# cheneeheng/2s-AGCN

Hardware: AMD Instinct MI355X
Metric: skeleton-clips/sec fwd+bwd, NTU (N,3,300,25,2) (higher is better)
Workload: dtype f32; 1 GPU; AGCN joint-stream NTU-xview shape, full training step (fwd, CE, bwd, grad all-reduce, clip 1.0, SGD nesterov); per_gpu_batch=64, global_batch=64, input=(N,3,300,25,2), parallelism=dp1, bn=per-replica

## Files before the change

### 2s-agcn_amd/csrc/conv_gemm_bf16.hip

```cpp
#include "agcn_common.h"
#include "epilogue.h"
#include "gate.h"
#include "split_f16.h"

namespace {

typedef __bf16 bf16x8 __attribute__((ext_vector_type(8)));
typedef __bf16 bf16x2 __attribute__((ext_vector_type(2)));
typedef float f32x2 __attribute__((ext_vector_type(2)));
typedef unsigned u32x4 __attribute__((ext_vector_type(4)));
typedef f32x4 f32x4_u __attribute__((aligned(4)));

constexpr int CK = 16, NW = 8, NT = 512;

struct BfArgs {
  const float* in;
  const unsigned short* wp;
  const float* bias;
  float* out;
  float* stats;
  const float* add1;
  const float* mask1;
  const float* add2;
  const float* mask2;
  int N, M, Kinner, in_rows;
  int V, T_src, T_out, tt, ntiles;
  int src_stride, f_off;
  int out_fs, out_fo, T_full;
  int FW, WLR;
  int accumulate;
  int nchunks, nmb;
  int off_b;
  int off_bias;
  int dbg;
  int relu;
  const float* in_absmax;
};

struct GateBfArgs : BfArgs {
  GateArgs gate;
  int off_gate;
};
template <bool GATE> struct BfArgsOf { typedef BfArgs type; };
template <> struct BfArgsOf<true> { typedef GateBfArgs type; };

struct BfPackArgs {
  const float* w;
  unsigned short* wp;
  int M, Kinner, nchunks;
  long sa_m, sa_c;
  int tap_mul, tap_add, tap_flip_from;
};

__device__ __forceinline__ unsigned pack_bf16(float a, float b) {
  f32x2 v = {a, b};
  bf16x2 p = __builtin_convertvector(v, bf16x2);
  return __builtin_bit_cast(unsigned, p);
}
__device__ __forceinline__ float lo_as_f32(unsigned p) { return __builtin_bit_cast(float, p << 16); }
__device__ __forceinline__ float hi_as_f32(unsigned p) { return __builtin_bit_cast(float, p & 0xffff0000u); }

__device__ __forceinline__ void split_pair(float a, float b, unsigned& ph, unsigned& pm, unsigned& pl) {
  ph = pack_bf16(a, b);
  const float ra = a - lo_as_f32(ph), rb = b - hi_as_f32(ph);
  pm = pack_bf16(ra, rb);
  pl = pack_bf16(ra - lo_as_f32(pm), rb - hi_as_f32(pm));
}

template <bool F16>
__device__ __forceinline__ f32x16 mfma_split(bf16x8 x, bf16x8 y, f32x16 c) {
  if constexpr (F16)
    return __builtin_amdgcn_mfma_f32_32x32x16_f16(__builtin_bit_cast(f16x8, x), __builtin_bit_cast(f16x8, y), c, 0, 0, 0);
  else
    return __builtin_amdgcn_mfma_f32_32x32x16_bf16(x, y, c, 0, 0, 0);
}

template <int TAPS, int BM, bool F16 = false>
__global__ void __launch_bounds__(256) pack_weights_bf16_kernel(const BfPackArgs p) {
  constexpr int PER_PLANE = TAPS * 2 * BM * 8;
  const int ch = blockIdx.x % p.nchunks, mb = blockIdx.x / p.nchunks;
  unsigned short* dst = p.wp + (long)blockIdx.x * 3 * PER_PLANE;
  for (int e = threadIdx.x; e < PER_PLANE / 2; e += 256) {
    const int j = (e & 3) * 2;
    const int ml = (e >> 2) % BM;
    const int r = (e >> 2) / BM;
    const int h = r & 1, tap = r >> 1;
    const int m = mb * BM + ml;
    const int gt = p.tap_flip_from >= 0 ? (p.tap_flip_from - (tap * p.tap_mul + p.tap_add)) : tap;
    float v[2];
#pragma unroll
    for (int q = 0; q < 2; ++q) {
      const int kc = ch * CK + h * 8 + j + q;
      v[q] = (m < p.M && kc < p.Kinner) ? p.w[(long)m * p.sa_m + (long)kc * p.sa_c + gt] : 0.f;
    }
    unsigned ph, pm, pl = 0;
    if constexpr (F16) split_pair_f16(v[0] * F16_W_SCALE, v[1] * F16_W_SCALE, ph, pm);
    else split_pair(v[0], v[1], ph, pm, pl);
    const int o = ((tap * 2 + h) * BM + ml) * 8 + j;
    *reinterpret_cast<unsigned*>(dst + 0 * PER_PLANE + o) = ph;
    *reinterpret_cast<unsigned*>(dst + 1 * PER_PLANE + o) = pm;
    *reinterpret_cast<unsigned*>(dst + 2 * PER_PLANE + o) = pl;
  }
}

template <int TAPS, int NPL, int WQ, int TM, int TN = 1, bool F16 = false, bool GATE = false>
__global__ void __launch_bounds__(NT, (TAPS == 1 && TM == 2 && TN == 1) ? 4 : 2) conv_gemm_bf16_kernel(const typename BfArgsOf<GATE>::type a) {
  constexpr int BM = TM * 32;
  constexpr int A_PLANE = TAPS * 2 * BM * 16;
  constexpr int A4 = NPL * A_PLANE / 16;
  constexpr int EA = (A4 + NT - 1) / NT;
  extern __shared__ __attribute__((aligned(16))) unsigned char smem[];
  unsigned char* Ab = smem;
  unsigned char* Bb = smem + a.off_b;

  const int tid = threadIdx.x, lane = tid & 63;
  const int wave = __builtin_amdgcn_readfirstlane(tid >> 6);
  const int lr = lane & 31, h = lane >> 5;
  const int bid = xcd_remap(blockIdx.x, gridDim.x);
  const int mbk = bid % a.nmb;
  const int nt_id = bid / a.nmb;
  const int n = nt_id / a.ntiles, tile_id = nt_id - n * a.ntiles;
  const int m0 = mbk * BM;
  const int V = a.V, tt = a.tt, t0 = tile_id * tt;
  const int ttv = tt * V;
  const int nvalid = min(tt, a.T_out - t0) * V;
  const int Psrc = a.T_src * V;
  const int f0 = t0 * a.src_stride + a.f_off;
  const int WL = a.FW * V, WLR = a.WLR;
  const int g0 = f0 * V;
  float rs_s = 1.f, rs_inv = 1.f;
  if constexpr (F16) { f16_range_scale(a.in_absmax, rs_s, rs_inv); rs_inv *= F16_W_INV; }

  int boff[TN];
#pragma unroll
  for (int tn = 0; tn < TN; ++tn) {
    int q = (wave * TN + tn) * 32 + lr;
    if (q >= ttv) q = 0;
    const int tl = q / V;
    boff[tn] = tl * a.src_stride * V + (q - tl * V);
  }

  float* bias_s = reinterpret_cast<float*>(smem + a.off_bias);
  for (int e = tid; e < BM; e += NT) bias_s[e] = (a.bias && m0 + e < a.M) ? a.bias[m0 + e] : 0.f;

  f32x16 acc[TM][TN];
#pragma unroll
  for (int tm = 0; tm < TM; ++tm)
#pragma unroll
    for (int tn = 0; tn < TN; ++tn)
#pragma unroll
      for (int j = 0; j < 16; ++j) acc[tm][tn][j] = 0.f;

  const int hb = wave & 1, wq = wave >> 1;
  const int qlen = (WL + 3) >> 2;
  u32x4 ra[EA];
  float rb[WQ][8];
  const int KP = a.nchunks * CK;
  const float* gl = nullptr;
  float gpos[WQ];
  if constexpr (GATE) {
    gl = reinterpret_cast<const float*>(smem + a.off_gate);
    gate_stage<NT>(reinterpret_cast<float*>(smem + a.off_gate), a.gate, n, V, a.T_src, a.Kinner, f0, a.FW, KP);
    __syncthreads();
#pragma unroll
    for (int u = 0; u < WQ; ++u) {
      const int rr = lane + 64 * u;
      gpos[u] = rr < qlen ? gate_pos(gl, KP, wq * qlen + rr, V, WL) : 0.f;
    }
    if constexpr (F16) {
      if (a.in_absmax) {
        f16_range_scale_of<14>(*a.in_absmax * gate_bound(gl, KP, a.FW, lane), rs_s, rs_inv);
        rs_inv *= F16_W_INV;
      }
    }
  }
  const u32x4* wp4 = reinterpret_cast<const u32x4*>(a.wp) + (long)mbk * a.nchunks * (3 * A_PLANE / 16);

  auto issue_loads = [&](int ch) __attribute__((always_inline)) {
    const u32x4* src = wp4 + (long)ch * (3 * A_PLANE / 16);
#pragma unroll
    for (int u = 0; u < EA; ++u) ra[u] = src[min(tid + u * NT, A4 - 1)];
    const int kc0 = ch * CK + hb * 8;
#pragma unroll
    for (int u = 0; u < WQ; ++u) {
      const int rr = lane + 64 * u;
      const int r = wq * qlen + rr;
      const int gp = g0 + r;
      const bool okp = rr < qlen && r < WL && gp >= 0 && gp < Psrc;
#pragma unroll
      for (int c = 0; c < 8; ++c) {
        const bool ok = okp && (kc0 + c) < a.Kinner;
        rb[u][c] = a.in[((long)n * a.in_rows + (ok ? (kc0 + c) : 0)) * Psrc + (ok ? gp : 0)];
      }
    }
  };
  auto commit_lds = [&](int ch) __attribute__((always_inline)) {
#pragma unroll
    for (int u = 0; u < EA; ++u)
      if (tid + u * NT < A4) reinterpret_cast<u32x4*>(Ab)[tid + u * NT] = ra[u];
    const int kc0 = ch * CK + hb * 8;
#pragma unroll
    for (int u = 0; u < WQ; ++u) {
      const int rr = lane + 64 * u;
      const int r = wq * qlen + rr;
      const int gp = g0 + r;
      const bool okp = rr < qlen && r < WL && gp >= 0 && gp < Psrc;
      u32x4 ph, pm, pl;
#pragma unroll
      for (int c = 0; c < 4; ++c) {
        float x0 = (okp && (kc0 + 2 * c) < a.Kinner) ? rb[u][2 * c] : 0.f;
        float x1 = (okp && (kc0 + 2 * c + 1) < a.Kinner) ? rb[u][2 * c + 1] : 0.f;
        if constexpr (GATE) {
          x0 = x0 * gpos[u] * gl[kc0 + 2 * c];
          x1 = x1 * gpos[u] * gl[kc0 + 2 * c + 1];
        }
        unsigned a0, a1, a2 = 0;
        if constexpr (F16) split_pair_f16(x0 * rs_s, x1 * rs_s, a0, a1);
        else split_pair(x0, x1, a0, a1, a2);
        ph[c] = a0; pm[c] = a1; pl[c] = a2;
      }
      if (rr < qlen && r < WL) {
        *reinterpret_cast<u32x4*>(Bb + ((0 * 2 + hb) * WLR + r) * 16) = ph;
        if (NPL >= 2) *reinterpret_cast<u32x4*>(Bb + ((1 * 2 + hb) * WLR + r) * 16) = pm;
        if (NPL == 3) *reinterpret_cast<u32x4*>(Bb + ((2 * 2 + hb) * WLR + r) * 16) = pl;
      }
    }
  };

  const int nchunks = a.nchunks;
  if (nchunks > 0) issue_loads(0);
  for (int ch = 0; ch < nchunks; ++ch) {
    __syncthreads();
    if (!(a.dbg & 2) || ch == 0) {
      commit_lds(ch);
      if (ch + 1 < nchunks) issue_loads(ch + 1);
    }
    __syncthreads();
    if (a.dbg & 1) continue;
    bf16x8 afc[NPL], bfc[NPL][TN];
    auto load_a = [&](bf16x8 (&af)[NPL], int tap, int tm) __attribute__((always_inline)) {
#pragma unroll
      for (int pl = 0; pl < NPL; ++pl)
        af[pl] = *reinterpret_cast<const bf16x8*>(Ab + pl * A_PLANE + (((tap * 2 + h) * BM) + tm * 32 + lr) * 16);
    };
    auto load_b = [&](bf16x8 (&bf)[NPL][TN], int tap) __attribute__((always_inline)) {
#pragma unroll
      for (int pl = 0; pl < NPL; ++pl)
#pragma unroll
        for (int tn = 0; tn < TN; ++tn)
          bf[pl][tn] = *reinterpret_cast<const bf16x8*>(Bb + ((pl * 2 + h) * WLR + boff[tn] + tap * V) * 16);
    };
    load_b(bfc, 0);
    load_a(afc, 0, 0);
    __builtin_amdgcn_sched_group_barrier(0x100, NPL * (TN + 1), 0);
#pragma unroll 1
    for (int tap = 0; tap < TAPS; ++tap) {
      bf16x8 bfn[NPL][TN];
      const int tapn = min(tap + 1, TAPS - 1);
#pragma unroll
      for (int tm = 0; tm < TM; ++tm) {
        bf16x8 afn[NPL];
        load_a(afn, tm + 1 == TM ? tapn : tap, tm + 1 == TM ? 0 : tm + 1);
        if (tm + 1 == TM) load_b(bfn, tapn);
#pragma unroll
        for (int tn = 0; tn < TN; ++tn) {
          if (NPL == 3) {
            acc[tm][tn] = mfma_split<F16>(afc[NPL - 1], bfc[0][tn], acc[tm][tn]);
            acc[tm][tn] = mfma_split<F16>(afc[0], bfc[NPL - 1][tn], acc[tm][tn]);
            acc[tm][tn] = mfma_split<F16>(afc[NPL >= 2 ? 1 : 0], bfc[NPL >= 2 ? 1 : 0][tn], acc[tm][tn]);
          }
          if (NPL >= 2) {
            acc[tm][tn] = mfma_split<F16>(afc[NPL >= 2 ? 1 : 0], bfc[0][tn], acc[tm][tn]);
            acc[tm][tn] = mfma_split<F16>(afc[0], bfc[NPL >= 2 ? 1 : 0][tn], acc[tm][tn]);
          }
          acc[tm][tn] = mfma_split<F16>(afc[0], bfc[0][tn], acc[tm][tn]);
        }
        __builtin_amdgcn_sched_group_barrier(0x100, NPL, 0);
        if (tm + 1 == TM) __builtin_amdgcn_sched_group_barrier(0x100, NPL * TN, 0);
        __builtin_amdgcn_sched_group_barrier(0x008, TN * (NPL == 3 ? 6 : NPL == 2 ? 3 : 1), 0);
#pragma unroll
        for (int pl = 0; pl < NPL; ++pl) afc[pl] = afn[pl];
      }
#pragma unroll
      for (int pl = 0; pl < NPL; ++pl)
#pragma unroll
        for (int tn = 0; tn < TN; ++tn) bfc[pl][tn] = bfn[pl][tn];
    }
  }

  if ((a.dbg & 4) && acc[0][0][0] != 12345.f) return;
  __syncthreads();
  float* tile = reinterpret_cast<float*>(smem);
  const int TP = NW * TN * 32 + 1;
  float* red = tile + BM * TP;
#pragma unroll
  for (int tm = 0; tm < TM; ++tm)
#pragma unroll
    for (int tn = 0; tn < TN; ++tn)
#pragma unroll
      for (int j = 0; j < 16; ++j)
        tile[(tm * 32 + mfma_row(j, h)) * TP + (wave * TN + tn) * 32 + lr] = F16 ? acc[tm][tn][j] * rs_inv : acc[tm][tn][j];
  __syncthreads();
  int poff[4 * TN];
#pragma unroll
  for (int u = 0; u < 4 * TN; ++u) {
    const int q2 = lane + 64 * u;
    const int tl2 = q2 / V;
    poff[u] = tl2 * a.out_fs * V + (q2 - tl2 * V);
  }
  EpiPtrs ep;
  ep.out = a.out; ep.add1 = a.add1; ep.mask1 = a.mask1; ep.add2 = a.add2; ep.mask2 = a.mask2; ep.stats = a.stats;
  ep.accumulate = a.accumulate; ep.relu = a.relu;
  const long Pfull = (long)a.T_full * V;
  const long rows0 = (long)n * a.M * Pfull + ((long)t0 * a.out_fs + a.out_fo) * V;
  epilogue_rows<BM, NW, 4 * TN>(ep, tile, TP, bias_s, red, a.M, m0, rows0, Pfull, nvalid, poff, (long)n * a.ntiles + tile_id);
}


template <int TAPS, int NPL, int R, int NWP = 4, bool F16 = false, bool GATE = false>
__global__ void __launch_bounds__((8 + NWP) * 64, 3) conv_pc_kernel(const typename BfArgsOf<GATE>::type a) {
  constexpr int TM = 4, BM = 128, NWC = 8, NTALL = (NWC + NWP) * 64, NTP = NWP * 64;
  constexpr int SLOT = NPL * 2 * BM * 16;
  constexpr int PIECES = SLOT / 1024;
  constexpr int PPW = (PIECES + NWP - 1) / NWP;
  constexpr int NMF = NPL == 3 ? 6 : NPL == 2 ? 3 : 1;
  extern __shared__ __attribute__((aligned(16))) unsigned char smem[];
  unsigned char* ring = smem;
  const int WLR = a.WLR, V = a.V;
  const int B_BYTES = NPL * 2 * WLR * 16;
  unsigned char* Bbase = smem + a.off_b;

  const int wave = __builtin_amdgcn_readfirstlane(threadIdx.x >> 6);
  const int lane = threadIdx.x & 63;
  const int bid = xcd_remap(blockIdx.x, gridDim.x);
  const int mbk = bid % a.nmb;
  const int nt_id = bid / a.nmb;
  const int n = nt_id / a.ntiles, tile_id = nt_id - n * a.ntiles;
  const int m0 = mbk * BM;
  const int tt = a.tt, t0 = tile_id * tt;
  const int ttv = tt * V;
  const int nvalid = min(tt, a.T_out - t0) * V;
  const int Psrc = a.T_src * V;
  const int g0 = (t0 + a.f_off) * V;
  const int WL = a.FW * V;
  const int nchunks = a.nchunks;
  const int G = nchunks * TAPS;
  float rs_s = 1.f, rs_inv = 1.f;
  if constexpr (F16) { f16_range_scale(a.in_absmax, rs_s, rs_inv); rs_inv *= F16_W_INV; }

  float* bias_s = reinterpret_cast<float*>(smem + a.off_bias);
  for (int e = threadIdx.x; e < BM; e += NTALL) bias_s[e] = (a.bias && m0 + e < a.M) ? a.bias[m0 + e] : 0.f;
  const int KP = nchunks * CK;
  const float* gl = nullptr;
  if constexpr (GATE) {
    gl = reinterpret_cast<const float*>(smem + a.off_gate);
    gate_stage<NTALL>(reinterpret_cast<float*>(smem + a.off_gate), a.gate, n, V, a.T_src, a.Kinner, t0 + a.f_off, a.FW, KP);
    __syncthreads();
    if constexpr (F16) {
      if (a.in_absmax) {
        f16_range_scale_of<14>(*a.in_absmax * gate_bound(gl, KP, a.FW, lane), rs_s, rs_inv);
        rs_inv *= F16_W_INV;
      }
    }
  }

  auto step_barrier = [&]() __attribute__((always_inline)) {
    asm volatile("s_waitcnt lgkmcnt(0)\n\ts_barrier" ::: "memory");
  };

  if (wave >= NWC) {
    const int pw = wave - NWC;
    typedef const __attribute__((address_space(1))) void* gptr_t;
    typedef __attribute__((address_space(3))) void* lptr_t;
    const unsigned char* wsrc = reinterpret_cast<const unsigned char*>(a.wp) + (long)mbk * G * SLOT + lane * 16;
    auto dma_slot = [&](int g) __attribute__((always_inline)) {
      const unsigned char* src = wsrc + (long)g * SLOT;
      unsigned char* dst = ring + (g % R) * SLOT;
#pragma unroll
      for (int u = 0; u < PPW; ++u) {
        const int piece = pw + u * NWP;
        if (piece < PIECES)
          __builtin_amdgcn_global_load_lds((gptr_t)(src + piece * 1024), (lptr_t)(dst + piece * 1024), 16, 0, 0);
      }
    };
    const int ptid = threadIdx.x - NWC * 64;
    const int npiece = (WL + 3) >> 2;
    const int ntask = 2 * npiece;
    constexpr int TK = 256 / NTP;
    f32x4 rb[TK][8];
    auto issue_B = [&](int ch) __attribute__((always_inline)) {
#pragma unroll
      for (int k = 0; k < TK; ++k) {
        if (k * NTP >= ntask) continue;
        int task = ptid + k * NTP;
        if (task >= ntask) task = ntask - 1;
        const int hb = task & 1, r0 = (task >> 1) * 4;
        const int gp = g0 + r0;
        const float* src = a.in + ((long)n * a.in_rows + ch * CK + hb * 8) * Psrc + gp;
        if (gp >= 0 && gp + 3 < Psrc) {
#pragma unroll
          for (int c = 0; c < 8; ++c) rb[k][c] = *reinterpret_cast<const f32x4_u*>(src + (long)c * Psrc);
        } else {
#pragma unroll
          for (int c = 0; c < 8; ++c)
#pragma unroll
            for (int e = 0; e < 4; ++e) {
              const bool ok = gp + e >= 0 && gp + e < Psrc;
              const float t = src[(long)c * Psrc + (ok ? e : -gp)];
              rb[k][c][e] = ok ? t : 0.f;
            }
        }
      }
    };
    float gpos[TK][4];
    if constexpr (GATE) {
#pragma unroll
      for (int k = 0; k < TK; ++k) {
        int task = ptid + k * NTP;
        if (task >= ntask) task = ntask - 1;
#pragma unroll
        for (int e = 0; e < 4; ++e) gpos[k][e] = (k * NTP < ntask) ? gate_pos(gl, KP, (task >> 1) * 4 + e, V, WL) : 0.f;
      }
    }
    auto commit_B = [&](unsigned char* Bb, int ch) __attribute__((always_inline)) {
#pragma unroll
      for (int k = 0; k < TK; ++k) {
        if (k * NTP >= ntask) continue;
        int task = ptid + k * NTP;
        if (task >= ntask) task = ntask - 1;
        const int hb = task & 1, r0 = (task >> 1) * 4;
        float gch[8];
        if constexpr (GATE) {
          const f32x4 g0v = *reinterpret_cast<const f32x4*>(gl + ch * CK + hb * 8);
          const f32x4 g1v = *reinterpret_cast<const f32x4*>(gl + ch * CK + hb * 8 + 4);
#pragma unroll
          for (int c = 0; c < 4; ++c) { gch[c] = g0v[c]; gch[4 + c] = g1v[c]; }
        }
#pragma unroll
        for (int e = 0; e < 4; ++e) {
          u32x4 ph, pm, pl;
#pragma unroll
          for (int c = 0; c < 4; ++c) {
            unsigned q0, q1, q2 = 0;
            float x0 = rb[k][2 * c][e], x1 = rb[k][2 * c + 1][e];
            if constexpr (GATE) {
              x0 = x0 * gpos[k][e] * gch[2 * c];
              x1 = x1 * gpos[k][e] * gch[2 * c + 1];
            }
            if constexpr (F16) split_pair_f16(x0 * rs_s, x1 * rs_s, q0, q1);
            else split_pair(x0, x1, q0, q1, q2);
            ph[c] = q0; pm[c] = q1; pl[c] = q2;
          }
          const int r = r0 + e;
          if (r < WLR) {
            *reinterpret_cast<u32x4*>(Bb + ((0 * 2 + hb) * WLR + r) * 16) = ph;
            if (NPL >= 2) *reinterpret_cast<u32x4*>(Bb + ((1 * 2 + hb) * WLR + r) * 16) = pm;
            if (NPL == 3) *reinterpret_cast<u32x4*>(Bb + ((2 * 2 + hb) * WLR + r) * 16) = pl;
          }
        }
      }
    };
#pragma unroll
    for (int g = 0; g < R - 1; ++g)
      if (g < G) dma_slot(g);
    issue_B(0);
    commit_B(Bbase, 0);
    asm volatile("s_waitcnt vmcnt(0)" ::: "memory");
    step_barrier();
    int g = 0;
    for (int ch = 0; ch < nchunks; ++ch) {
#pragma unroll
      for (int tap = 0; tap < TAPS; ++tap, ++g) {
        if (a.dbg & 2) { step_barrier(); continue; }
        if (g + R - 1 < G && !(a.dbg & 8)) dma_slot(g + R - 1);
        if (TAPS >= 3) {
          if (tap == 0 && ch + 1 < nchunks && !(a.dbg & 4)) issue_B(ch + 1);
          if (tap == (TAPS >= 6 ? TAPS - 3 : TAPS - 2) && ch + 1 < nchunks && !(a.dbg & 4))
            commit_B(Bbase + ((ch + 1) & 1) * B_BYTES, ch + 1);
        } else {
          if (tap == 0 && ch + 1 < nchunks) { issue_B(ch + 1); commit_B(Bbase + ((ch + 1) & 1) * B_BYTES, ch + 1); }
        }
        if (g + R - 1 < G) asm volatile("s_waitcnt vmcnt(%0)" :: "n"(PPW * (R - 3)) : "memory");
        else asm volatile("s_waitcnt vmcnt(0)" ::: "memory");
        step_barrier();
      }
    }
    return;
  }

  const int lr = lane & 31, h = lane >> 5;
  int q = wave * 32 + lr;
  if (q >= ttv) q = 0;
  const int boff = q;
  f32x16 acc[TM];
#pragma unroll
  for (int tm = 0; tm < TM; ++tm)
#pragma unroll
    for (int j = 0; j < 16; ++j) acc[tm][j] = 0.f;

  const unsigned char* a_lane = ring + (h * BM + lr) * 16;
  auto load_a = [&](bf16x8 (&af)[NPL], int slot, int tm) __attribute__((always_inline)) {
#pragma unroll
    for (int pl = 0; pl < NPL; ++pl)
      af[pl] = *reinterpret_cast<const bf16x8*>(a_lane + slot * SLOT + (pl * 2 * BM + tm * 32) * 16);
  };
  auto load_b = [&](bf16x8 (&bf)[NPL], const unsigned char* Bb, int tap) __attribute__((always_inline)) {
#pragma unroll
    for (int pl = 0; pl < NPL; ++pl)
      bf[pl] = *reinterpret_cast<const bf16x8*>(Bb + ((pl * 2 + h) * WLR + boff + tap * V) * 16);
  };
  step_barrier();
  bf16x8 afc[NPL], bfc[NPL];
  load_b(bfc, Bbase, 0);
  load_a(afc, 0, 0);
  int slot = 0;
  for (int ch = 0; ch < nchunks; ++ch) {
    const unsigned char* Bb = Bbase + (ch & 1) * B_BYTES;
    const unsigned char* Bn = Bbase + ((ch + 1) & 1) * B_BYTES;
#pragma unroll
    for (int tap = 0; tap < TAPS; ++tap) {
      const int slot_n = (slot + 1 == R) ? 0 : slot + 1;
      if (a.dbg & 1) { step_barrier(); continue; }
      bf16x8 bfn[NPL];
#pragma unroll
      for (int tm = 0; tm < TM; ++tm) {
        bf16x8 afn[NPL];
        if (tm + 1 < TM) {
          load_a(afn, slot, tm + 1);
        } else {
          load_a(afn, slot_n, 0);
          if (tap + 1 < TAPS) load_b(bfn, Bb, tap + 1);
          else load_b(bfn, Bn, 0);
        }
        if (NPL == 3) {
          acc[tm] = mfma_split<F16>(afc[NPL - 1], bfc[0], acc[tm]);
          acc[tm] = mfma_split<F16>(afc[0], bfc[NPL - 1], acc[tm]);
          acc[tm] = mfma_split<F16>(afc[NPL >= 2 ? 1 : 0], bfc[NPL >= 2 ? 1 : 0], acc[tm]);
        }
        if (NPL >= 2) {
          acc[tm] = mfma_split<F16>(afc[NPL >= 2 ? 1 : 0], bfc[0], acc[tm]);
          acc[tm] = mfma_split<F16>(afc[0], bfc[NPL >= 2 ? 1 : 0], acc[tm]);
        }
        acc[tm] = mfma_split<F16>(afc[0], bfc[0], acc[tm]);
        __builtin_amdgcn_sched_group_barrier(0x100, NPL, 0);
        if (tm + 1 == TM) __builtin_amdgcn_sched_group_barrier(0x100, NPL, 0);
        __builtin_amdgcn_sched_group_barrier(0x008, NMF, 0);
#pragma unroll
        for (int pl = 0; pl < NPL; ++pl) afc[pl] = afn[pl];
      }
#pragma unroll
      for (int pl = 0; pl < NPL; ++pl) bfc[pl] = bfn[pl];
      slot = slot_n;
      step_barrier();
    }
  }

  float* tile = reinterpret_cast<float*>(smem);
  const int TP = NWC * 32 + 1;
  float* red = tile + BM * TP;
#pragma unroll
  for (int tm = 0; tm < TM; ++tm)
#pragma unroll
    for (int j = 0; j < 16; ++j) tile[(tm * 32 + mfma_row(j, h)) * TP + wave * 32 + lr] = F16 ? acc[tm][j] * rs_inv : acc[tm][j];
  __syncthreads();
  int poff[4];
#pragma unroll
  for (int u = 0; u < 4; ++u) {
    const int q2 = lane + 64 * u;
    const int tl2 = q2 / V;
    poff[u] = tl2 * a.out_fs * V + (q2 - tl2 * V);
  }
  EpiPtrs ep;
  ep.out = a.out; ep.add1 = a.add1; ep.mask1 = a.mask1; ep.add2 = a.add2; ep.mask2 = a.mask2; ep.stats = a.stats;
  ep.accumulate = a.accumulate; ep.relu = a.relu;
  const long Pfull = (long)a.T_full * V;
  const long rows0 = (long)n * a.M * Pfull + ((long)t0 * a.out_fs + a.out_fo) * V;
  epilogue_rows<BM, NWC, 4>(ep, tile, TP, bias_s, red, a.M, m0, rows0, Pfull, nvalid, poff, (long)n * a.ntiles + tile_id);
}

template <int TAPS, int BM, int NPL, bool F16 = false>
__global__ void __launch_bounds__(256) pack_weights_slots_kernel(const BfPackArgs p) {
  constexpr int PLANE = 2 * BM * 8;
  const int tap = blockIdx.x % TAPS;
  const int ch = (blockIdx.x / TAPS) % p.nchunks, mb = blockIdx.x / (TAPS * p.nchunks);
  unsigned short* dst = p.wp + (long)blockIdx.x * NPL * PLANE;
  const int gt = p.tap_flip_from >= 0 ? (p.tap_flip_from - (tap * p.tap_mul + p.tap_add)) : tap;
  for (int e = threadIdx.x; e < PLANE / 2; e += 256) {
    const int j = (e & 3) * 2;
    const int ml = (e >> 2) % BM;
    const int h = (e >> 2) / BM;
    const int m = mb * BM + ml;
    float v[2];
#pragma unroll
    for (int q = 0; q < 2; ++q) {
      const int kc = ch * CK + h * 8 + j + q;
      v[q] = (m < p.M && kc < p.Kinner) ? p.w[(long)m * p.sa_m + (long)kc * p.sa_c + gt] : 0.f;
    }
    unsigned ph, pm, pl = 0;
    if constexpr (F16) split_pair_f16(v[0] * F16_W_SCALE, v[1] * F16_W_SCALE, ph, pm);
    else split_pair(v[0], v[1], ph, pm, pl);
    const int o = (h * BM + ml) * 8 + j;
    *reinterpret_cast<unsigned*>(dst + 0 * PLANE + o) = ph;
    if (NPL >= 2) *reinterpret_cast<unsigned*>(dst + 1 * PLANE + o) = pm;
    if (NPL == 3) *reinterpret_cast<unsigned*>(dst + 2 * PLANE + o) = pl;
  }
}

struct BfGeom {
  int tt, ntiles, FW, WLR, nchunks, nmb, off_b, off_bias;
  size_t smem_bytes, pack_bytes;
};

template <int TAPS, int BM, int TN = 1>
BfGeom bf_geometry(int V, int T_out, int src_stride, int M, int Kinner) {
  BfGeom g;
  g.tt = (256 * TN) / V;
  if (g.tt > T_out) g.tt = T_out;
  if (g.tt < 1) g.tt = 1;
  g.ntiles = (T_out + g.tt - 1) / g.tt;
  g.FW = (g.tt - 1) * src_stride + TAPS;
  g.WLR = g.FW * V + 8;
  g.nchunks = (Kinner + CK - 1) / CK;
  g.nmb = (M + BM - 1) / BM;
  const size_t a_bytes = (size_t)3 * TAPS * 2 * BM * 16;
  g.off_b = (int)a_bytes;
  const size_t b_bytes = (size_t)3 * 2 * g.WLR * 16;
  size_t main_b = a_bytes + b_bytes;
  size_t epi_b = (size_t)BM * (NW * TN * 32 + 1) * 4 + (size_t)NT * 2 * 4;
  g.smem_bytes = ((main_b > epi_b ? main_b : epi_b) + 15) & ~(size_t)15;
  g.off_bias = (int)g.smem_bytes;
  g.smem_bytes += (size_t)BM * 4;
  g.pack_bytes = (size_t)g.nmb * g.nchunks * a_bytes;
  return g;
}

struct BfProblem {
  BfArgs a;
  GateArgs gate;
  int fwd_f16;
  const float* w;
  long sa_m, sa_c;
  int tap_mul, tap_add, tap_flip_from;
  void* ws;
  size_t ws_bytes;
  int stats_tiles;
};

inline size_t gate_bytes(const BfGeom& g) { return 4 * (size_t)gate_lds_floats(g.FW, g.nchunks * CK); }

template <int TAPS, int NPL, int WQ, int TM, int TN = 1, bool F16 = false, bool GATE = false>
int launch_bf(BfProblem& p, hipStream_t stream) {
  constexpr int BM = TM * 32;
  typename BfArgsOf<GATE>::type a;
  static_cast<BfArgs&>(a) = p.a;
  BfGeom g = bf_geometry<TAPS, BM, TN>(a.V, a.T_out, a.src_stride, a.M, a.Kinner);
  if constexpr (GATE) {
    a.gate = p.gate;
    a.off_gate = (int)g.smem_bytes;
    g.smem_bytes += gate_bytes(g);
  }
  if (g.smem_bytes > 160 * 1024) return AGCN_ERR_UNSUPPORTED;
  if ((g.FW * a.V + 3) / 4 > WQ * 64) return AGCN_ERR_UNSUPPORTED;
  if (g.pack_bytes > p.ws_bytes) return AGCN_ERR_WORKSPACE;
  if (a.stats && p.stats_tiles > 0 && g.ntiles != p.stats_tiles) return AGCN_ERR_ARG;
  a.tt = g.tt; a.ntiles = g.ntiles; a.FW = g.FW; a.WLR = g.WLR; a.nchunks = g.nchunks; a.nmb = g.nmb;
  a.off_b = g.off_b; a.off_bias = g.off_bias;
  a.wp = (const unsigned short*)p.ws;
  static const int dbg = getenv("AGCN_CB_DBG") ? atoi(getenv("AGCN_CB_DBG")) : 0;
  a.dbg = dbg;
  if (g.nchunks > 0) {
    BfPackArgs pk;
    pk.w = p.w; pk.wp = (unsigned short*)p.ws; pk.M = a.M; pk.Kinner = a.Kinner; pk.nchunks = g.nchunks;
    pk.sa_m = p.sa_m; pk.sa_c = p.sa_c;
    pk.tap_mul = p.tap_mul; pk.tap_add = p.tap_add; pk.tap_flip_from = p.tap_flip_from;
    hipLaunchKernelGGL((pack_weights_bf16_kernel<TAPS, BM, F16>), dim3(g.nmb * g.nchunks), dim3(256), 0, stream, pk);
    int rc = agcn_check_launch();
    if (rc) return rc;
  }
  auto kern = conv_gemm_bf16_kernel<TAPS, NPL, WQ, TM, TN, F16, GATE>;
  static unsigned char lds_ok[AGCN_MAX_DEVICES] = {};
  if (int e = agcn_allow_big_lds_rt(reinterpret_cast<const void*>(kern), lds_ok)) return e;
  if (GATE) AGCN_NOTE_KERNEL("conv_gemm_bf16_kernel<%d, %d, %d, %d, %d, %s, true> [gates on load]", TAPS, NPL, WQ, TM, TN, F16 ? "true" : "false");
  else AGCN_NOTE_KERNEL("conv_gemm_bf16_kernel<%d, %d, %d, %d, %d, %s>", TAPS, NPL, WQ, TM, TN, F16 ? "true" : "false");
  hipLaunchKernelGGL(kern, dim3((unsigned)(a.N * g.ntiles * g.nmb)), dim3(NT), g.smem_bytes, stream, a);
  return agcn_check_launch();
}


template <int TAPS, int NPL, int R>
BfGeom bf_geometry_pc(int V, int T_out, int M, int Kinner) {
  constexpr int BM = 128, SLOT = NPL * 2 * BM * 16;
  BfGeom g;
  g.tt = 256 / V;
  if (g.tt > T_out) g.tt = T_out;
  if (g.tt < 1) g.tt = 1;
  g.ntiles = (T_out + g.tt - 1) / g.tt;
  g.FW = (g.tt - 1) + TAPS;
  g.WLR = g.FW * V + 8;
  g.nchunks = (Kinner + CK - 1) / CK;
  g.nmb = (M + BM - 1) / BM;
  g.off_b = R * SLOT;
  const size_t main_b = (size_t)g.off_b + 2 * (size_t)NPL * 2 * g.WLR * 16;
  const size_t epi_b = (size_t)BM * (8 * 32 + 1) * 4 + (size_t)512 * 2 * 4;
  g.smem_bytes = ((main_b > epi_b ? main_b : epi_b) + 15) & ~(size_t)15;
  g.off_bias = (int)g.smem_bytes;
  g.smem_bytes += (size_t)BM * 4;
  g.pack_bytes = (size_t)g.nmb * g.nchunks * TAPS * SLOT;
  return g;
}

static inline bool conv_pc_enabled() {
  static int v = -1;
  if (v < 0) {
    const char* e = getenv("AGCN_CONV_PC");
    v = (e && atoi(e) == 0) ? 0 : 1;
  }
  return v == 1;
}

template <int TAPS, int NPL, int R = 5, int NWP = 4, bool F16 = false, bool GATE = false>
int launch_pc(BfProblem& p, hipStream_t stream) {
  constexpr int BM = 128;
  typename BfArgsOf<GATE>::type a;
  static_cast<BfArgs&>(a) = p.a;
  BfGeom g = bf_geometry_pc<TAPS, NPL, R>(a.V, a.T_out, a.M, a.Kinner);
  if constexpr (GATE) {
    a.gate = p.gate;
    a.off_gate = (int)g.smem_bytes;
    g.smem_bytes += gate_bytes(g);
  }
  if (g.smem_bytes > 160 * 1024) return AGCN_ERR_UNSUPPORTED;
  if (g.pack_bytes > p.ws_bytes) return AGCN_ERR_WORKSPACE;
  if (a.stats && p.stats_tiles > 0 && g.ntiles != p.stats_tiles) return AGCN_ERR_ARG;
  a.tt = g.tt; a.ntiles = g.ntiles; a.FW = g.FW; a.WLR = g.WLR; a.nchunks = g.nchunks; a.nmb = g.nmb;
  a.off_b = g.off_b; a.off_bias = g.off_bias;
  a.wp = (const unsigned short*)p.ws;
  BfPackArgs pk;
  pk.w = p.w; pk.wp = (unsigned short*)p.ws; pk.M = a.M; pk.Kinner = a.Kinner; pk.nchunks = g.nchunks;
  pk.sa_m = p.sa_m; pk.sa_c = p.sa_c;
  pk.tap_mul = p.tap_mul; pk.tap_add = p.tap_add; pk.tap_flip_from = p.tap_flip_from;
  hipLaunchKernelGGL((pack_weights_slots_kernel<TAPS, BM, NPL, F16>), dim3(g.nmb * g.nchunks * TAPS), dim3(256), 0, stream, pk);
  int rc = agcn_check_launch();
  if (rc) return rc;
  auto kern = conv_pc_kernel<TAPS, NPL, R, NWP, F16, GATE>;
  static unsigned char lds_ok[AGCN_MAX_DEVICES] = {};
  if (int e = agcn_allow_big_lds_rt(reinterpret_cast<const void*>(kern), lds_ok)) return e;
  static const int dbg = getenv("AGCN_CB_DBG") ? atoi(getenv("AGCN_CB_DBG")) : 0;
  a.dbg = dbg;
  if (GATE) AGCN_NOTE_KERNEL("conv_pc_kernel<%d, %d, %d, %d, %s, true> [gates on load]", TAPS, NPL, R, NWP, F16 ? "true" : "false");
  else AGCN_NOTE_KERNEL("conv_pc_kernel<%d, %d, %d, %d, %s>", TAPS, NPL, R, NWP, F16 ? "true" : "false");
  hipLaunchKernelGGL(kern, dim3((unsigned)(a.N * g.ntiles * g.nmb)), dim3((8 + NWP) * 64), g.smem_bytes, stream, a);
  return agcn_check_launch();
}

template <int TAPS>
bool pc_applies(const BfProblem& p, int npl, bool gate = false) {
  if (!conv_pc_enabled() || TAPS < 3 || npl != 3) return false;
  if (p.a.M % 128 != 0 || p.a.Kinner % CK != 0 || p.a.src_stride != 1 || p.a.V > 32) return false;
  const BfGeom g = bf_geometry_pc<TAPS, 3, 5>(p.a.V, p.a.T_out, p.a.M, p.a.Kinner);
  return g.smem_bytes + (gate ? gate_bytes(g) : 0) <= 160 * 1024 && g.FW * p.a.V <= 512;
}

template <int TAPS, int WQ, bool GATE = false>
int launch_npl(BfProblem& p, int npl, hipStream_t s) {
  const BfGeom g128 = bf_geometry<TAPS, 128>(p.a.V, p.a.T_out, p.a.src_stride, p.a.M, p.a.Kinner);
  const bool fits128 = g128.smem_bytes + (GATE ? gate_bytes(g128) : 0) <= 160 * 1024;
  if constexpr (TAPS >= 3) {
    if (pc_applies<TAPS>(p, npl, GATE)) {
      static const int nwp2 = getenv("AGCN_CONV_NWP2") ? atoi(getenv("AGCN_CONV_NWP2")) : 0;
      if (nwp2 && !GATE) return launch_pc<TAPS, 3, 5, 2>(p, s);
      if (p.fwd_f16) return launch_pc<TAPS, 2, 5, 4, true, GATE>(p, s);
      return launch_pc<TAPS, 3, 5, 4, false, GATE>(p, s);
    }
  }
  if constexpr (TAPS >= 3) {
    if (p.fwd_f16) {
      if (p.a.M % 128 == 0 && fits128) return launch_bf<TAPS, 2, WQ, 4, 1, true, GATE>(p, s);
      if (agcn_bf16_conv_wide(TAPS, p.a.M)) {
        const int rc = launch_bf<TAPS, 2, 3, 2, 2, true, GATE>(p, s);
        if (rc != AGCN_ERR_UNSUPPORTED) return rc;
      }
      return launch_bf<TAPS, 2, WQ, 2, 1, true, GATE>(p, s);
    }
  }
  if (p.a.M % 128 == 0 && fits128) {
    if (npl == 1) return launch_bf<TAPS, 1, WQ, 4, 1, false, GATE>(p, s);
    return npl == 2 ? launch_bf<TAPS, 2, WQ, 4, 1, false, GATE>(p, s) : launch_bf<TAPS, 3, WQ, 4, 1, false, GATE>(p, s);
  }
  if (agcn_bf16_conv_wide(TAPS, p.a.M) && (npl == 3 || npl == 1)) {
    const int rc = npl == 3 ? launch_bf<TAPS, 3, 3, 2, 2, false, GATE>(p, s) : launch_bf<TAPS, 1, 3, 2, 2, false, GATE>(p, s);
    if (rc != AGCN_ERR_UNSUPPORTED) return rc;
  }
  if (npl == 1) return launch_bf<TAPS, 1, WQ, 2, 1, false, GATE>(p, s);
  return npl == 2 ? launch_bf<TAPS, 2, WQ, 2, 1, false, GATE>(p, s) : launch_bf<TAPS, 3, WQ, 2, 1, false, GATE>(p, s);
}

}

bool agcn_bf16_conv_wide(int taps, int M) {
  static int v = -1;
  if (v < 0) {
    const char* e = getenv("AGCN_CONV_WIDE");
    v = (e && atoi(e) == 0) ? 0 : 1;
  }
  return v == 1 && taps > 1 && M <= 64;
}

size_t agcn_bf16_conv_workspace(int Cin, int Cout, int T, int V, int stride) {
  const int To = (T + 8 - 9) / stride + 1;
  size_t b = bf_geometry<9, 64>(V, To, stride, Cout, Cin).pack_bytes, t;
  t = bf_geometry<9, 64>(V, T, 1, Cin, Cout).pack_bytes; if (t > b) b = t;
  t = bf_geometry<9, 128>(V, To, stride, Cout, Cin).pack_bytes; if (t > b) b = t;
  t = bf_geometry<9, 128>(V, T, 1, Cin, Cout).pack_bytes; if (t > b) b = t;
  return b + 256;
}

namespace {

int bf16_in_absmax(BfProblem& p, const float* given, const float* in, long n, hipStream_t s) {
  if (given) {
    p.a.in_absmax = given;
    return 0;
  }
  if (p.ws_bytes < 64) return AGCN_ERR_WORKSPACE;
  unsigned* amax = reinterpret_cast<unsigned*>(static_cast<char*>(p.ws) + ((p.ws_bytes - 16) & ~(size_t)15));
  if (hipMemsetAsync(amax, 0, 4, s) != hipSuccess) return AGCN_ERR_ARG;
  hipLaunchKernelGGL(absmax_kernel, dim3(2048), dim3(256), 0, s, in, n, amax);
  if (int rc = agcn_check_launch()) return rc;
  p.a.in_absmax = reinterpret_cast<const float*>(amax);
  p.ws_bytes = (p.ws_bytes - 16) & ~(size_t)15;
  return 0;
}

int bf16_fwd_f16x3(int npl) {
  static const int f16x3 = getenv("AGCN_CONV_F16X3") ? atoi(getenv("AGCN_CONV_F16X3")) : 1;
  return f16x3 && npl == 3;
}

template <int TAPS, int WQ, bool GATE = false>
int bf16_tconv_fwd(const float* x, const float* w, const float* bias, float* y, float* stats_part, void* ws,
                   size_t ws_bytes, int N, int Cin, int Cout, int T, int V, int stride, int pad, int npl, hipStream_t s,
                   const float* add, int relu, const float* x_absmax, const GateArgs* gate = nullptr) {
  BfProblem p = {};
  BfArgs& a = p.a;
  a.in = x; a.bias = bias; a.out = y; a.stats = stats_part; a.add1 = add; a.relu = relu;
  if (GATE) p.gate = *gate;
  p.fwd_f16 = bf16_fwd_f16x3(npl);
  p.ws = ws; p.ws_bytes = ws_bytes;
  if (p.fwd_f16)
    if (int rc = bf16_in_absmax(p, x_absmax, x, (long)N * Cin * T * V, s)) return rc;
  a.N = N; a.M = Cout; a.Kinner = Cin; a.in_rows = Cin; a.V = V;
  a.T_src = T; a.T_out = (T + 2 * pad - TAPS) / stride + 1; a.T_full = a.T_out;
  a.src_stride = stride; a.f_off = -pad; a.out_fs = 1; a.out_fo = 0;
  p.w = w; p.sa_m = (long)Cin * TAPS; p.sa_c = TAPS; p.tap_flip_from = -1;
  if (TAPS != 9 && stats_part) {
    const int tt = agcn_bf16_tconv_tile_frames(TAPS, Cout, V, a.T_out, npl);
    p.stats_tiles = (a.T_out + tt - 1) / tt;
  }
  return launch_npl<TAPS, WQ, GATE>(p, npl, s);
}

template <int TAPS>
int bf16_tconv_bwd_data_s1(const float* dy, const float* w, float* dx, int accumulate, const float* add1,
                           const float* mask1, const float* add2, const float* mask2, void* ws, size_t ws_bytes, int N,
                           int Cin, int Cout, int T, int V, int pad, int npl, hipStream_t s, const float* dy_absmax) {
  BfProblem p = {};
  BfArgs& a = p.a;
  p.fwd_f16 = bf16_fwd_f16x3(npl);
  p.ws = ws; p.ws_bytes = ws_bytes;
  const int To = T + 2 * pad - TAPS + 1;
  if (p.fwd_f16)
    if (int rc = bf16_in_absmax(p, dy_absmax, dy, (long)N * Cout * To * V, s)) return rc;
  a.in = dy; a.out = dx; a.accumulate = accumulate;
  a.add1 = add1; a.mask1 = mask1; a.add2 = add2; a.mask2 = mask2;
  a.N = N; a.M = Cin; a.Kinner = Cout; a.in_rows = Cout; a.V = V;
  a.T_src = To; a.T_full = T; a.src_stride = 1;
  a.T_out = T; a.out_fs = 1; a.out_fo = 0; a.f_off = pad - (TAPS - 1);
  p.w = w; p.sa_m = TAPS; p.sa_c = (long)Cin * TAPS;
  p.tap_mul = 1; p.tap_add = 0; p.tap_flip_from = TAPS - 1;
  return launch_npl<TAPS, 2>(p, npl, s);
}

}

int agcn_bf16_conv9_fwd(const float* x, const float* w, const float* bias, float* y, float* stats_part, void* ws,
                        size_t ws_bytes, int N, int Cin, int Cout, int T, int V, int stride, int npl,
                        hipStream_t s, const float* add, int relu, const float* x_absmax) {
  if (stride == 1)
    return bf16_tconv_fwd<9, 2>(x, w, bias, y, stats_part, ws, ws_bytes, N, Cin, Cout, T, V, 1, 4, npl, s, add, relu,
                                x_absmax);
  return bf16_tconv_fwd<9, 3>(x, w, bias, y, stats_part, ws, ws_bytes, N, Cin, Cout, T, V, stride, 4, npl, s, add, relu,
                              x_absmax);
}

int agcn_bf16_conv9_bwd_data(const float* dy, const float* w, float* dx, int accumulate, const float* add1,
                             const float* mask1, const float* add2, const float* mask2, void* ws, size_t ws_bytes,
                             int N, int Cin, int Cout, int T, int V, int stride, int npl, hipStream_t s,
                             const float* dy_absmax) {
  if (stride == 1)
    return bf16_tconv_bwd_data_s1<9>(dy, w, dx, accumulate, add1, mask1, add2, mask2, ws, ws_bytes, N, Cin, Cout, T, V,
                                     4, npl, s, dy_absmax);
  BfProblem p = {};
  BfArgs& a = p.a;
  p.fwd_f16 = bf16_fwd_f16x3(npl);
  p.ws = ws; p.ws_bytes = ws_bytes;
  if (p.fwd_f16)
    if (int rc = bf16_in_absmax(p, dy_absmax, dy, (long)N * Cout * ((T + 8 - 9) / stride + 1) * V, s)) return rc;
  a.in = dy; a.out = dx; a.accumulate = accumulate;
  a.add1 = add1; a.mask1 = mask1; a.add2 = add2; a.mask2 = mask2;
  a.N = N; a.M = Cin; a.Kinner = Cout; a.in_rows = Cout; a.V = V;
  a.T_src = (T + 8 - 9) / stride + 1; a.T_full = T; a.src_stride = 1;
  p.w = w; p.sa_m = 9; p.sa_c = (long)Cin * 9;
  a.T_out = (T + 1) / 2; a.out_fs = 2; a.out_fo = 0; a.f_off = -2;
  p.tap_mul = 2; p.tap_add = 0; p.tap_flip_from = 8;
  int rc = launch_npl<5, 2>(p, npl, s);
  if (rc) return rc;
  a.T_out = T / 2; a.out_fo = 1; a.f_off = -1;
  p.tap_add = 1;
  if (a.T_out > 0) rc = launch_npl<4, 2>(p, npl, s);
  return rc;
}

bool agcn_bf16_tconv_supported(int taps, int stride) { return stride == 1 && (taps == 3 || taps == 5 || taps == 7); }

int agcn_bf16_tconv_fwd(const float* x, const float* w, const float* bias, float* y, float* stats_part, void* ws,
                        size_t ws_bytes, int N, int Cin, int Cout, int T, int V, int taps, int pad, int npl,
                        hipStream_t s, const float* x_absmax) {
  switch (taps) {
    case 3: return bf16_tconv_fwd<3, 2>(x, w, bias, y, stats_part, ws, ws_bytes, N, Cin, Cout, T, V, 1, pad, npl, s,
                                        nullptr, 0, x_absmax);
    case 5: return bf16_tconv_fwd<5, 2>(x, w, bias, y, stats_part, ws, ws_bytes, N, Cin, Cout, T, V, 1, pad, npl, s,
                                        nullptr, 0, x_absmax);
    case 7: return bf16_tconv_fwd<7, 2>(x, w, bias, y, stats_part, ws, ws_bytes, N, Cin, Cout, T, V, 1, pad, npl, s,
                                        nullptr, 0, x_absmax);
    default: return AGCN_ERR_UNSUPPORTED;
  }
}

int agcn_bf16_tconv_bwd_data(const float* dy, const float* w, float* dx, int accumulate, const float* add1,
                             const float* mask1, const float* add2, const float* mask2, void* ws, size_t ws_bytes,
                             int N, int Cin, int Cout, int T, int V, int taps, int pad, int npl, hipStream_t s,
                             const float* dy_absmax) {
  switch (taps) {
    case 3: return bf16_tconv_bwd_data_s1<3>(dy, w, dx, accumulate, add1, mask1, add2, mask2, ws, ws_bytes, N, Cin, Cout,
                                             T, V, pad, npl, s, dy_absmax);
    case 5: return bf16_tconv_bwd_data_s1<5>(dy, w, dx, accumulate, add1, mask1, add2, mask2, ws, ws_bytes, N, Cin, Cout,
                                             T, V, pad, npl, s, dy_absmax);
    case 7: return bf16_tconv_bwd_data_s1<7>(dy, w, dx, accumulate, add1, mask1, add2, mask2, ws, ws_bytes, N, Cin, Cout,
                                             T, V, pad, npl, s, dy_absmax);
    default: return AGCN_ERR_UNSUPPORTED;
  }
}

template <int TAPS, int WQ>
static int bf16_tconv_infer_t(const float* x, const float* w, const float* bias, float* y, void* ws, size_t ws_bytes, int N,
                              int Cin, int Cout, int T, int V, int stride, int pad, int npl, hipStream_t s,
                              const float* add, int relu, const float* x_absmax, const GateArgs* gate) {
  const bool gated = gate && (gate->gs || gate->gt || gate->gc);
  {
    const int To = (T + 2 * pad - TAPS) / stride + 1;
    const BfGeom g = bf_geometry<TAPS, 64>(V, To, stride, Cout, Cin);
    if (g.smem_bytes + (gated ? gate_bytes(g) : 0) > 160 * 1024 || (g.FW * V + 3) / 4 > WQ * 64) return AGCN_ERR_UNSUPPORTED;
  }
  if (gated)
    return bf16_tconv_fwd<TAPS, WQ, true>(x, w, bias, y, nullptr, ws, ws_bytes, N, Cin, Cout, T, V, stride, pad, npl, s, add,
                                          relu, x_absmax, gate);
  return bf16_tconv_fwd<TAPS, WQ>(x, w, bias, y, nullptr, ws, ws_bytes, N, Cin, Cout, T, V, stride, pad, npl, s, add, relu,
                                  x_absmax);
}

bool agcn_bf16_tconv_infer_supported(int taps, int stride, int pad) {
  if (taps == 9) return pad == 4 && (stride == 1 || stride == 2);
  return agcn_bf16_tconv_supported(taps, stride);
}

int agcn_bf16_tconv_infer(const float* x, const float* w, const float* bias, float* y, void* ws, size_t ws_bytes, int N,
                          int Cin, int Cout, int T, int V, int taps, int stride, int pad, int npl, hipStream_t s,
                          const float* add, int relu, const float* x_absmax, const GateArgs* gate) {
  if (!agcn_bf16_tconv_infer_supported(taps, stride, pad)) return AGCN_ERR_UNSUPPORTED;
#define AGCN_INFER_CASE(TAPS, WQ) \
  return bf16_tconv_infer_t<TAPS, WQ>(x, w, bias, y, ws, ws_bytes, N, Cin, Cout, T, V, stride, pad, npl, s, add, relu, x_absmax, gate)
  switch (taps) {
    case 3: AGCN_INFER_CASE(3, 2);
    case 5: AGCN_INFER_CASE(5, 2);
    case 7: AGCN_INFER_CASE(7, 2);
    default: break;
  }
  if (stride == 1) AGCN_INFER_CASE(9, 2);
  AGCN_INFER_CASE(9, 3);
#undef AGCN_INFER_CASE
}

int agcn_bf16_tconv_tile_frames(int taps, int M, int V, int T_out, int npl) {
  int tt = 256 / V;
  if (M <= 64 && agcn_bf16_conv_wide(taps, M) && (npl == 3 || npl == 1)) {
    bool ok = false;
    switch (taps) {
      case 3: ok = bf_geometry<3, 64, 2>(V, T_out, 1, M, 16).smem_bytes <= 160 * 1024; break;
      case 5: ok = bf_geometry<5, 64, 2>(V, T_out, 1, M, 16).smem_bytes <= 160 * 1024; break;
      case 7: ok = bf_geometry<7, 64, 2>(V, T_out, 1, M, 16).smem_bytes <= 160 * 1024; break;
      default: break;
    }
    int tw = 512 / V;
    if (tw > T_out) tw = T_out;
    if (ok && ((tw - 1) + taps) * V <= 3 * 64 * 4) tt = 512 / V;
  }
  if (tt > T_out) tt = T_out;
  if (tt < 1) tt = 1;
  return tt;
}

int agcn_bf16_conv1_fwd(const float* x, const float* w, const float* bias, float* y, float* stats_part, void* ws,
                        size_t ws_bytes, int N, int Cin, int Cout, int T, int V, int stride, int npl,
                        hipStream_t s, const float* add, int relu) {
  BfProblem p = {};
  BfArgs& a = p.a;
  a.in = x; a.bias = bias; a.out = y; a.stats = stats_part; a.add1 = add; a.relu = relu;
  a.N = N; a.M = Cout; a.Kinner = Cin; a.in_rows = Cin; a.V = V;
  a.T_src = T; a.T_out = (T - 1) / stride + 1; a.T_full = a.T_out;
  a.src_stride = stride; a.f_off = 0; a.out_fs = 1; a.out_fo = 0;
  p.w = w; p.sa_m = Cin; p.sa_c = 1; p.tap_flip_from = -1;
  p.ws = ws; p.ws_bytes = ws_bytes;
  if (stride == 1) return launch_npl<1, 2>(p, npl, s);
  return launch_npl<1, 3>(p, npl, s);
}

int agcn_bf16_conv1_bwd_data(const float* dy, const float* w, float* dx, int accumulate, const float* add1,
                             const float* mask1, const float* add2, const float* mask2, void* ws, size_t ws_bytes,
                             int N, int Cin, int Cout, int T, int V, int npl, hipStream_t s) {
  BfProblem p = {};
  BfArgs& a = p.a;
  a.in = dy; a.out = dx; a.accumulate = accumulate;
  a.add1 = add1; a.mask1 = mask1; a.add2 = add2; a.mask2 = mask2;
  a.N = N; a.M = Cin; a.Kinner = Cout; a.in_rows = Cout; a.V = V;
  a.T_src = T; a.T_full = T; a.src_stride = 1;
  a.T_out = T; a.out_fs = 1; a.out_fo = 0; a.f_off = 0;
  p.w = w; p.sa_m = 1; p.sa_c = Cin; p.tap_mul = 1; p.tap_add = 0; p.tap_flip_from = 0;
  p.ws = ws; p.ws_bytes = ws_bytes;
  return launch_npl<1, 2>(p, npl, s);
}

size_t agcn_bf16_conv1_workspace(int Cin, int Cout, int T, int V, int stride) {
  const int To = (T - 1) / stride + 1;
  size_t b = bf_geometry<1, 64>(V, To, stride, Cout, Cin).pack_bytes, t;
  t = bf_geometry<1, 64>(V, T, 1, Cin, Cout).pack_bytes; if (t > b) b = t;
  t = bf_geometry<1, 128>(V, To, stride, Cout, Cin).pack_bytes; if (t > b) b = t;
  t = bf_geometry<1, 128>(V, T, 1, Cin, Cout).pack_bytes; if (t > b) b = t;
  return b + 256;
}
```

Measured before the change: 1015 clips/s.

## Add stride-2 producer/consumer conv path by splitting frames into even/odd parity

Extends the warp-specialized producer/consumer temporal conv kernel to stride-2 9-tap convolutions. The loaded window is stored as even frames followed by odd frames with a padded vertex pitch, and the weight slots are reordered as (2s mod TAPS), so each tap reads a contiguous stride-1 window. Stride-2 convs in the f16 forward path (the downsampling layers) now use the pipelined kernel instead of the generic bf16 path. The cost is a larger LDS window, a B staging load spread across two taps, and extra address arithmetic.

After: 1014 clips/s (median of 2 runs). About the same (-0.1%).

```diff
diff --git a/2s-agcn_amd/csrc/conv_gemm_bf16.hip b/2s-agcn_amd/csrc/conv_gemm_bf16.hip
--- a/2s-agcn_amd/csrc/conv_gemm_bf16.hip
+++ b/2s-agcn_amd/csrc/conv_gemm_bf16.hip
@@ -317,9 +317,11 @@
 }
 
 
-template <int TAPS, int NPL, int R, int NWP = 4, bool F16 = false, bool GATE = false>
+template <int TAPS, int NPL, int R, int NWP = 4, bool F16 = false, bool GATE = false, bool S2 = false>
 __global__ void __launch_bounds__((8 + NWP) * 64, 3) conv_pc_kernel(const typename BfArgsOf<GATE>::type a) {
   constexpr int TM = 4, BM = 128, NWC = 8, NTALL = (NWC + NWP) * 64, NTP = NWP * 64;
+  constexpr int TE = (TAPS + 1) / 2;
+  static_assert(!S2 || !GATE, "the gate vectors are laid out for a stride-1 window");
   constexpr int SLOT = NPL * 2 * BM * 16;
   constexpr int PIECES = SLOT / 1024;
   constexpr int PPW = (PIECES + NWP - 1) / NWP;
@@ -342,7 +344,8 @@
   const int nvalid = min(tt, a.T_out - t0) * V;
   const int Psrc = a.T_src * V;
   const int g0 = (t0 + a.f_off) * V;
-  const int WL = a.FW * V;
+  const int VP = S2 ? (V + 3) & ~3 : V;
+  const int WL = a.FW * VP;
   const int nchunks = a.nchunks;
   const int G = nchunks * TAPS;
   float rs_s = 1.f, rs_inv = 1.f;
@@ -386,16 +389,30 @@
     const int ptid = threadIdx.x - NWC * 64;
     const int npiece = (WL + 3) >> 2;
     const int ntask = 2 * npiece;
-    constexpr int TK = 256 / NTP;
+    constexpr int TK = S2 ? 2 : 256 / NTP;
     f32x4 rb[TK][8];
-    auto issue_B = [&](int ch) __attribute__((always_inline)) {
+    int gps[TK];
+    if constexpr (S2) {
+      const int ppf = VP >> 2, FE = tt - 1 + TE;
+#pragma unroll
+      for (int k = 0; k < TK; ++k) {
+        int task = ptid + k * NTP;
+        if (task >= ntask) task = ntask - 1;
+        const int piece = task >> 1;
+        const int j = piece / ppf;
+        const int f = 2 * t0 + a.f_off + (j < FE ? 2 * j : 2 * (j - FE) + 1);
+        gps[k] = f * V + (piece - j * ppf) * 4;
+      }
+    }
+    auto issue_B = [&](int ch, int only) __attribute__((always_inline)) {
 #pragma unroll
       for (int k = 0; k < TK; ++k) {
         if (k * NTP >= ntask) continue;
+        if (only >= 0 && k != only) continue;
         int task = ptid + k * NTP;
         if (task >= ntask) task = ntask - 1;
         const int hb = task & 1, r0 = (task >> 1) * 4;
-        const int gp = g0 + r0;
+        const int gp = S2 ? gps[k] : g0 + r0;
         const float* src = a.in + ((long)n * a.in_rows + ch * CK + hb * 8) * Psrc + gp;
         if (gp >= 0 && gp + 3 < Psrc) {
 #pragma unroll
@@ -463,7 +480,7 @@
 #pragma unroll
     for (int g = 0; g < R - 1; ++g)
       if (g < G) dma_slot(g);
-    issue_B(0);
+    issue_B(0, -1);
     commit_B(Bbase, 0);
     asm volatile("s_waitcnt vmcnt(0)" ::: "memory");
     step_barrier();
@@ -474,11 +491,11 @@
         if (a.dbg & 2) { step_barrier(); continue; }
         if (g + R - 1 < G && !(a.dbg & 8)) dma_slot(g + R - 1);
         if (TAPS >= 3) {
-          if (tap == 0 && ch + 1 < nchunks && !(a.dbg & 4)) issue_B(ch + 1);
+          if ((S2 ? tap < TK : tap == 0) && ch + 1 < nchunks && !(a.dbg & 4)) issue_B(ch + 1, S2 ? tap : -1);
           if (tap == (TAPS >= 6 ? TAPS - 3 : TAPS - 2) && ch + 1 < nchunks && !(a.dbg & 4))
             commit_B(Bbase + ((ch + 1) & 1) * B_BYTES, ch + 1);
         } else {
-          if (tap == 0 && ch + 1 < nchunks) { issue_B(ch + 1); commit_B(Bbase + ((ch + 1) & 1) * B_BYTES, ch + 1); }
+          if (tap == 0 && ch + 1 < nchunks) { issue_B(ch + 1, -1); commit_B(Bbase + ((ch + 1) & 1) * B_BYTES, ch + 1); }
         }
         if (g + R - 1 < G) asm volatile("s_waitcnt vmcnt(%0)" :: "n"(PPW * (R - 3)) : "memory");
         else asm volatile("s_waitcnt vmcnt(0)" ::: "memory");
@@ -491,7 +508,8 @@
   const int lr = lane & 31, h = lane >> 5;
   int q = wave * 32 + lr;
   if (q >= ttv) q = 0;
-  const int boff = q;
+  const int boff = S2 ? (q / V) * VP + q % V : q;
+  const int odd_off = (tt - 1) * VP;
   f32x16 acc[TM];
 #pragma unroll
   for (int tm = 0; tm < TM; ++tm)
@@ -507,7 +525,7 @@
   auto load_b = [&](bf16x8 (&bf)[NPL], const unsigned char* Bb, int tap) __attribute__((always_inline)) {
 #pragma unroll
     for (int pl = 0; pl < NPL; ++pl)
-      bf[pl] = *reinterpret_cast<const bf16x8*>(Bb + ((pl * 2 + h) * WLR + boff + tap * V) * 16);
+      bf[pl] = *reinterpret_cast<const bf16x8*>(Bb + ((pl * 2 + h) * WLR + boff + tap * VP + (S2 && tap >= TE ? odd_off : 0)) * 16);
   };
   step_barrier();
   bf16x8 afc[NPL], bfc[NPL];
@@ -584,7 +602,8 @@
   const int tap = blockIdx.x % TAPS;
   const int ch = (blockIdx.x / TAPS) % p.nchunks, mb = blockIdx.x / (TAPS * p.nchunks);
   unsigned short* dst = p.wp + (long)blockIdx.x * NPL * PLANE;
-  const int gt = p.tap_flip_from >= 0 ? (p.tap_flip_from - (tap * p.tap_mul + p.tap_add)) : tap;
+  const int gt = p.tap_flip_from >= 0 ? (p.tap_flip_from - (tap * p.tap_mul + p.tap_add))
+                                      : (p.tap_mul > 1 ? (tap * p.tap_mul + p.tap_add) % TAPS : tap);
   for (int e = threadIdx.x; e < PLANE / 2; e += 256) {
     const int j = (e & 3) * 2;
     const int ml = (e >> 2) % BM;
@@ -688,15 +707,15 @@
 
 
 template <int TAPS, int NPL, int R>
-BfGeom bf_geometry_pc(int V, int T_out, int M, int Kinner) {
+BfGeom bf_geometry_pc(int V, int T_out, int M, int Kinner, int src_stride = 1) {
   constexpr int BM = 128, SLOT = NPL * 2 * BM * 16;
   BfGeom g;
   g.tt = 256 / V;
   if (g.tt > T_out) g.tt = T_out;
   if (g.tt < 1) g.tt = 1;
   g.ntiles = (T_out + g.tt - 1) / g.tt;
-  g.FW = (g.tt - 1) + TAPS;
-  g.WLR = g.FW * V + 8;
+  g.FW = (g.tt - 1) * src_stride + TAPS;
+  g.WLR = g.FW * (src_stride == 2 ? (V + 3) & ~3 : V) + 8;
   g.nchunks = (Kinner + CK - 1) / CK;
   g.nmb = (M + BM - 1) / BM;
   g.off_b = R * SLOT;
@@ -718,12 +737,14 @@
   return v == 1;
 }
 
-template <int TAPS, int NPL, int R = 5, int NWP = 4, bool F16 = false, bool GATE = false>
+template <int TAPS, int NPL, int R = 5, int NWP = 4, bool F16 = false, bool GATE = false, bool S2 = false>
 int launch_pc(BfProblem& p, hipStream_t stream) {
   constexpr int BM = 128;
   typename BfArgsOf<GATE>::type a;
   static_cast<BfArgs&>(a) = p.a;
-  BfGeom g = bf_geometry_pc<TAPS, NPL, R>(a.V, a.T_out, a.M, a.Kinner);
+  if (a.src_stride != (S2 ? 2 : 1)) return AGCN_ERR_ARG;
+  BfGeom g = bf_geometry_pc<TAPS, NPL, R>(a.V, a.T_out, a.M, a.Kinner, a.src_stride);
+  if (g.WLR - 8 > (S2 ? 1024 : 512)) return AGCN_ERR_UNSUPPORTED;
   if constexpr (GATE) {
     a.gate = p.gate;
     a.off_gate = (int)g.smem_bytes;
@@ -739,15 +760,21 @@
   pk.w = p.w; pk.wp = (unsigned short*)p.ws; pk.M = a.M; pk.Kinner = a.Kinner; pk.nchunks = g.nchunks;
   pk.sa_m = p.sa_m; pk.sa_c = p.sa_c;
   pk.tap_mul = p.tap_mul; pk.tap_add = p.tap_add; pk.tap_flip_from = p.tap_flip_from;
+  if constexpr (S2) {
+    static_assert(TAPS % 2 == 1, "the slot order (2 s) mod TAPS needs an odd tap count");
+    if (p.tap_flip_from >= 0) return AGCN_ERR_ARG;
+    pk.tap_mul = 2; pk.tap_add = 0;
+  }
   hipLaunchKernelGGL((pack_weights_slots_kernel<TAPS, BM, NPL, F16>), dim3(g.nmb * g.nchunks * TAPS), dim3(256), 0, stream, pk);
   int rc = agcn_check_launch();
   if (rc) return rc;
-  auto kern = conv_pc_kernel<TAPS, NPL, R, NWP, F16, GATE>;
+  auto kern = conv_pc_kernel<TAPS, NPL, R, NWP, F16, GATE, S2>;
   static unsigned char lds_ok[AGCN_MAX_DEVICES] = {};
   if (int e = agcn_allow_big_lds_rt(reinterpret_cast<const void*>(kern), lds_ok)) return e;
   static const int dbg = getenv("AGCN_CB_DBG") ? atoi(getenv("AGCN_CB_DBG")) : 0;
   a.dbg = dbg;
   if (GATE) AGCN_NOTE_KERNEL("conv_pc_kernel<%d, %d, %d, %d, %s, true> [gates on load]", TAPS, NPL, R, NWP, F16 ? "true" : "false");
+  else if (S2) AGCN_NOTE_KERNEL("conv_pc_kernel<%d, %d, %d, %d, %s, false, true> [stride 2 by frame parity]", TAPS, NPL, R, NWP, F16 ? "true" : "false");
   else AGCN_NOTE_KERNEL("conv_pc_kernel<%d, %d, %d, %d, %s>", TAPS, NPL, R, NWP, F16 ? "true" : "false");
   hipLaunchKernelGGL(kern, dim3((unsigned)(a.N * g.ntiles * g.nmb)), dim3((8 + NWP) * 64), g.smem_bytes, stream, a);
   return agcn_check_launch();
@@ -759,6 +786,14 @@
   if (p.a.M % 128 != 0 || p.a.Kinner % CK != 0 || p.a.src_stride != 1 || p.a.V > 32) return false;
   const BfGeom g = bf_geometry_pc<TAPS, 3, 5>(p.a.V, p.a.T_out, p.a.M, p.a.Kinner);
   return g.smem_bytes + (gate ? gate_bytes(g) : 0) <= 160 * 1024 && g.FW * p.a.V <= 512;
+}
+
+template <int TAPS>
+bool pc_s2_applies(const BfProblem& p, int npl, bool gate) {
+  if (!conv_pc_enabled() || TAPS != 9 || npl != 3 || !p.fwd_f16 || gate || p.tap_flip_from >= 0) return false;
+  if (p.a.M % 128 != 0 || p.a.Kinner % CK != 0 || p.a.src_stride != 2 || p.a.V > 32) return false;
+  const BfGeom g = bf_geometry_pc<TAPS, 2, 5>(p.a.V, p.a.T_out, p.a.M, p.a.Kinner, 2);
+  return g.smem_bytes <= 160 * 1024 && g.WLR - 8 <= 1024;
 }
 
 template <int TAPS, int WQ, bool GATE = false>
@@ -772,6 +807,9 @@
       if (p.fwd_f16) return launch_pc<TAPS, 2, 5, 4, true, GATE>(p, s);
       return launch_pc<TAPS, 3, 5, 4, false, GATE>(p, s);
     }
+  }
+  if constexpr (TAPS == 9 && !GATE) {
+    if (pc_s2_applies<TAPS>(p, npl, GATE)) return launch_pc<TAPS, 2, 5, 4, true, false, true>(p, s);
   }
   if constexpr (TAPS >= 3) {
     if (p.fwd_f16) {
```
